# marcelodallaqua/TensorDiffEq

Measured on AMD Instinct MI355X. Metric: collocation-pts/sec + L2 rel-error, Allen-Cahn SA-PINN @ 1/2/4/8 GPU, higher is better.
Workload: dtype bf16; 1 GPU; model=Allen-Cahn SA-PINN tanh MLP [2,128,128,128,128,1], problem=ac-sa, global_batch=50000, parallelism=dp1, points_per_gpu=50000, backend=hip, bc_points=IC 512 (SA) + periodic 2x201 (u, u_x)

## Files before the change

tensordiffeq_amd/csrc/jet_bf3.hip:

```cpp
#include "jet_fused3.h"
#include "optim_common.h"

__device__ __forceinline__ void pack_frag(const float* __restrict__ P, bf16x8* __restrict__ img, const NetDims& d,
                                          int WT, int transposed, int e) {
  const int KB = WT / 2;
  {
    const int lane = e & 63, frag = e >> 6;
    const int kb = frag % KB, o = (frag / KB) % WT, layer = frag / (KB * WT) + 1;
    const int p = lane & 15, g = lane >> 4, row = 16 * o + p;
    const float* K = P + off_layer(d, layer);
    bf16x8 hi, lo;
#pragma unroll
    for (int j = 0; j < 8; ++j) {
      const int kf = 32 * kb + (j < 4 ? 4 * g + j : 16 + 4 * g + j - 4);
      const int in = transposed ? kf : row, out = transposed ? row : kf;
      const int win = hw(d, layer - 1), wout = hw(d, layer);
      const float v = (in < win && out < wout) ? K[in * wout + out] : 0.f;
      const __bf16 h = (__bf16)v;
      hi[j] = h;
      lo[j] = (__bf16)(v - (float)h);
    }
    img[(size_t)(frag * 2) * 64 + lane] = hi;
    img[(size_t)(frag * 2 + 1) * 64 + lane] = lo;
  }
}

__device__ __forceinline__ void pack_aux(const float* __restrict__ P, float* __restrict__ aux, const NetDims& d,
                                         int W, int e) {
  {
    float v = 0.f;
    const int w0 = hw(d, 0), wl = hw(d, d.n_hidden - 1);
    if (e < aux_b0(d, W)) {
      const int j = e / W, f = e - j * W;
      if (f < w0) v = P[j * w0 + f];
    } else if (e < aux_bh(d, W)) {
      const int f = e - aux_b0(d, W);
      if (f < w0) v = P[d.d_in * w0 + f];
    } else if (e < aux_ko(d, W)) {
      const int r = e - aux_bh(d, W), i = r / W + 1, f = r - (i - 1) * W;
      if (f < hw(d, i)) v = P[off_layer(d, i) + hw(d, i - 1) * hw(d, i) + f];
    } else if (e < aux_bo(d, W)) {
      const int r = e - aux_ko(d, W), f = r >> 2, q = r & 3;
      if (f < wl && q < d.d_out) v = P[off_layer(d, d.n_hidden) + f * d.d_out + q];
    } else {
      const int q = e - aux_bo(d, W);
      if (q < d.d_out) v = P[off_layer(d, d.n_hidden) + wl * d.d_out + q];
    }
    aux[e] = v;
  }
}

__global__ void __launch_bounds__(256) pack_all_kernel(const float* __restrict__ P, bf16x8* __restrict__ fimg,
                                                       bf16x8* __restrict__ bimg, float* __restrict__ aux, NetDims d,
                                                       int WT) {
  const int nf = (d.n_hidden - 1) * WT * (WT / 2) * 64;
  const int total = 2 * nf + aux_floats(d, 16 * WT);
  for (int e = blockIdx.x * 256 + threadIdx.x; e < total; e += gridDim.x * 256) {
    if (e < nf)
      pack_frag(P, fimg, d, WT, 1, e);
    else if (e < 2 * nf)
      pack_frag(P, bimg, d, WT, 0, e - nf);
    else
      pack_aux(P, aux, d, 16 * WT, e - 2 * nf);
  }
}

struct TailBook {
  const float* lpart;
  int n_lblocks, n_terms, n_scal;
  float* losses;
  float* total;
  float* dscal;
  float* hist;
  int64_t hist_rows;
  int64_t* epoch;
  float* best_loss;
  int64_t* best_epoch;
  int* improved;
  Counters cnt;
};

__global__ void __launch_bounds__(256) tail_reduce1_kernel(const float* __restrict__ slab, float* __restrict__ part,
                                                           int nwg, int Pst, int chunks, int nqb, int half, int c0,
                                                           TailBook tb) {
  if ((int)blockIdx.x < nqb) {
    const int q = blockIdx.x * 256 + threadIdx.x, c = c0 + (int)blockIdx.y;
    if (half) {
      if (8 * q < Pst) slab_reduce1_body8(slab, part, nwg, Pst, chunks, q, c);
    } else if (4 * q < Pst) {
      slab_reduce1_body<false>(slab, part, nwg, Pst, chunks, q, c);
    }
    return;
  }
  if (blockIdx.y != 0) return;
  __shared__ float sh[256];
  const int ns = tb.n_terms + tb.n_scal;
  for (int slot = 0; slot < ns; ++slot) {
    float s = 0.f;
    for (int b = threadIdx.x; b < tb.n_lblocks; b += 256) s += tb.lpart[(size_t)b * ns + slot];
    sh[threadIdx.x] = s;
    __syncthreads();
    for (int k = 128; k > 0; k >>= 1) {
      if ((int)threadIdx.x < k) sh[threadIdx.x] += sh[threadIdx.x + k];
      __syncthreads();
    }
    if (threadIdx.x == 0) {
      if (slot < tb.n_terms) tb.losses[slot] = sh[0];
      else tb.dscal[slot - tb.n_terms] = sh[0];
    }
    __syncthreads();
  }
  if (threadIdx.x == 0 && tb.hist == nullptr && tb.total != nullptr) {
    float s = 0.f;
    for (int t = 0; t < tb.n_terms; ++t) s += tb.losses[t];
    *tb.total = s;
  }
  if (threadIdx.x == 0 && tb.hist != nullptr)
    step_book_body(tb.total, tb.losses, tb.n_terms, 1, tb.hist, tb.hist_rows, tb.epoch, tb.best_loss, tb.best_epoch,
                   tb.improved, tb.cnt);
}

__global__ void __launch_bounds__(256) slab_reduce2_bf3(const float* __restrict__ part, float* __restrict__ grad, int P,
                                                        int Pst, int chunks, const float* __restrict__ gx) {
  const int q = blockIdx.x * 256 + threadIdx.x;
  if (4 * q >= P) return;
  const f32x4 a = slab_reduce2_sum(part, Pst, chunks, q);
#pragma unroll
  for (int e = 0; e < 4; ++e)
    if (4 * q + e < P) grad[4 * q + e] = gx != nullptr ? a[e] + gx[4 * q + e] : a[e];
}

__global__ void __launch_bounds__(256) tail_adam_kernel(AdamArgs args, const float* __restrict__ part, int Pst,
                                                        int chunks, const int* __restrict__ improved,
                                                        float* __restrict__ snap, TailImg ti,
                                                        const float* __restrict__ gx) {
  const bool do_snap = snap != nullptr && *improved != 0;
  const int64_t total = args.start[args.ngroups];
  for (int64_t idx = (int64_t)blockIdx.x * 256 + threadIdx.x; idx < total; idx += (int64_t)gridDim.x * 256) {
    const int gi = adam_group_of(args, idx);
    const AdamGroup gr = args.grp[gi];
    const int64_t e = idx - args.start[gi];
    const bool th = gi == 0;
    float g;
    if (th && part != nullptr) {
      float a0 = 0.f, a1 = 0.f;
      int c = 0;
      for (; c + 7 < chunks; c += 8) {
        float v[8];
#pragma unroll
        for (int k = 0; k < 8; ++k) v[k] = part[(size_t)(c + k) * Pst + e];
#pragma unroll
        for (int k = 0; k < 8; k += 2) {
          a0 += v[k];
          a1 += v[k + 1];
        }
      }
      for (; c + 1 < chunks; c += 2) {
        a0 += part[(size_t)c * Pst + e];
        a1 += part[(size_t)(c + 1) * Pst + e];
      }
      if (c < chunks) a0 += part[(size_t)c * Pst + e];
      g = a0 + a1;
      if (gx != nullptr) g += gx[e];
      const_cast<float*>(gr.g)[e] = g;
    } else {
      g = gr.g[e];
    }
    float p = gr.p[e], m = gr.m[e], v = gr.v[e];
    if (do_snap && th) snap[e] = p;
    adam_elem(p, gr.sign * g, m, v, gr.b1, gr.b2, gr.eps, adam_lr_t(gr));
    gr.p[e] = p;
    gr.m[e] = m;
    gr.v[e] = v;
    if (th && ti.fimg != nullptr) scatter_param(p, (int)e, ti);
  }
}

namespace {

int64_t img_floats(int WT, int n_hidden) {
  return (int64_t)(n_hidden > 1 ? n_hidden - 1 : 0) * WT * (WT / 2) * 128 * 4;
}

int64_t aux_alloc(int d_in, int n_hidden, int W) { return ((int64_t)(d_in + n_hidden + 4) * W + 4 + 3) / 4 * 4; }

int64_t stage_floats(int N, int WT, int S, int lo) {
  const int64_t nwg = (N + 63) / 64;
  return bf3_gstage(WT, S, lo != 0) ? nwg * 4 * stage_wave_elems(WT, S, true) * 2 : 0;
}

int bf3_rows(int N, const NetDims& d, int WT, int S, int lo) {
  const int pts_b = 16 * bwd_waves(WT, lo != 0, S);
  return (N + pts_b - 1) / pts_b;
}

int launch_pack(const float* P, bf16x8* fimg, bf16x8* bimg, float* aux, NetDims d, int WT, hipStream_t st) {
  const int total = 2 * (d.n_hidden - 1) * WT * (WT / 2) * 64 + aux_floats(d, 16 * WT);
  int blocks = (total + 255) / 256;
  if (blocks > 1024) blocks = 1024;
  hipLaunchKernelGGL(pack_all_kernel, dim3(blocks), dim3(256), 0, st, P, fimg, bimg, aux, d, WT);
  TDQ_CHECK_LAUNCH();
  return 0;
}

bool bf3_ok(int WT, int S, int d_in, int d_out, int n_hidden) {
  return (WT == 2 || WT == 4 || WT == 8 || (WT == 16 && S <= 4)) && S >= 1 && S <= TDQ_MAXS &&
         d_in <= TDQ_MAXD && d_out <= TDQ_MAXO && n_hidden >= 1;
}

int dispatch(bool fwd, int WT, int S, int nso, const Bf3Args& a) {
  switch (WT) {
    case 2: return fwd ? bf3_fwd_w2(S, nso, a) : bf3_bwd_w2(S, nso, a);
    case 4: return fwd ? bf3_fwd_w4(S, nso, a) : bf3_bwd_w4(S, nso, a);
    case 8: return fwd ? bf3_fwd_w8(S, nso, a) : bf3_bwd_w8(S, nso, a);
    case 16: return fwd ? bf3_fwd_w16(S, nso, a) : bf3_bwd_w16(S, nso, a);
    default: return (int)hipErrorInvalidValue;
  }
}

}

extern "C" {

int64_t tdq_jet_bf3_scratch_floats(int N, int d_in, const int* widths, int n_hidden, int S, int lo) {
  NetDims d;
  if (!make_dims(d, d_in, widths, 0, 1, n_hidden)) return -1;
  const int WT = width_tiles(d.width);
  if (WT < 2) return -1;
  const int64_t nwg = (N + 63) / 64;
  const int64_t hs = (int64_t)n_hidden * nwg * S * 4 * WT * 256;
  return hs + 2 * img_floats(WT, n_hidden) + aux_alloc(d_in, n_hidden, 16 * WT) + stage_floats(N, WT, S, lo);
}

int64_t tdq_jet_bf3_slab_floats(int N, int d_in, const int* widths, int d_out, int n_hidden) {
  NetDims d;
  if (!make_dims(d, d_in, widths, 0, d_out, n_hidden)) return -1;
  const int WT = width_tiles(d.width);
  if (WT < 2) return -1;
  int nwg = (N + 63) / 64;
  const int fz = (N + 15) / 16 < fz_cus() ? (N + 15) / 16 : fz_cus();
  if (fz > nwg) nwg = fz;
  const int64_t P = slab_stride(param_count(d));
  return ((int64_t)nwg + slab_chunks(nwg)) * P;
}

int64_t tdq_slab_floats_rows(int rows, int d_in, const int* widths, int d_out, int n_hidden) {
  NetDims d;
  if (rows < 1 || !make_dims(d, d_in, widths, 0, d_out, n_hidden)) return -1;
  return ((int64_t)rows + slab_chunks(rows)) * slab_stride(param_count(d));
}

static inline void scratch_images(float* scratch, int n_hidden, int WT, float** img, float** bimg, float** aux) {
  *img = scratch;
  *bimg = *img + img_floats(WT, n_hidden);
  *aux = *bimg + img_floats(WT, n_hidden);
}

static inline bf16x4* scratch_stage(float* scratch, int N, int d_in, int n_hidden, int S, int WT, int lo) {
  if (!bf3_gstage(WT, S, lo != 0)) return nullptr;
  float *img, *bimg, *aux;
  scratch_images(scratch, n_hidden, WT, &img, &bimg, &aux);
  return reinterpret_cast<bf16x4*>(aux + aux_alloc(d_in, n_hidden, 16 * WT));
}

static inline float* scratch_hs(float* scratch, int N, int d_in, int n_hidden, int S, int WT, int lo) {
  return scratch + 2 * img_floats(WT, n_hidden) + aux_alloc(d_in, n_hidden, 16 * WT) + stage_floats(N, WT, S, lo);
}

int tdq_jet_fwd_bf3_range(const float* X, const float* P, float* J, float* scratch, int N, int p_lo, int p_hi,
                          int d_in, const int* widths, int d_out, int n_hidden, int S, const int* spec, int lo, int pack,
                          void* stream) {
  if (N <= 0) return 0;
  if (p_lo < 0 || p_lo % 128 != 0 || p_hi > N || p_hi <= p_lo || (p_hi != N && p_hi % 128 != 0))
    return (int)hipErrorInvalidValue;
  NetDims d;
  if (!make_dims(d, d_in, widths, 0, d_out, n_hidden)) return (int)hipErrorInvalidValue;
  const int WT = width_tiles(d.width);
  JetSpec sp;
  if (!bf3_ok(WT, S, d_in, d_out, n_hidden)) return (int)hipErrorInvalidValue;
  const int nso = spec_nso(S, spec);
  if (nso < 0 || !make_spec(S, spec, sp)) return (int)hipErrorInvalidValue;
  hipStream_t st = reinterpret_cast<hipStream_t>(stream);
  float* Hs = scratch_hs(scratch, N, d_in, n_hidden, S, WT, lo);
  float *img, *bimg, *aux;
  scratch_images(scratch, n_hidden, WT, &img, &bimg, &aux);
  if (pack) {
    int rc = launch_pack(P, reinterpret_cast<bf16x8*>(img), reinterpret_cast<bf16x8*>(bimg), aux, d, WT, st);
    if (rc) return rc;
  }
  Bf3Args a{X, aux, reinterpret_cast<const bf16x8*>(img), nullptr, J, Hs, nullptr, N, 0, d, sp, st, lo,
            scratch_stage(scratch, N, d_in, n_hidden, S, WT, lo), p_lo, p_hi};
  return dispatch(true, WT, S, nso, a);
}

int tdq_jet_fwd_bf3_ex(const float* X, const float* P, float* J, float* scratch, int N, int d_in, const int* widths,
                       int d_out, int n_hidden, int S, const int* spec, int lo, int pack, void* stream) {
  return tdq_jet_fwd_bf3_range(X, P, J, scratch, N, 0, N, d_in, widths, d_out, n_hidden, S, spec, lo, pack, stream);
}

int tdq_jet_fwd_bf3(const float* X, const float* P, float* J, float* scratch, int N, int d_in, const int* widths,
                    int d_out, int n_hidden, int S, const int* spec, int lo, void* stream) {
  return tdq_jet_fwd_bf3_ex(X, P, J, scratch, N, d_in, widths, d_out, n_hidden, S, spec, lo, 1, stream);
}

int tdq_jet_bf3_pack(const float* P, float* scratch, int N, int d_in, const int* widths, int d_out, int n_hidden, int S,
                     void* stream) {
  NetDims d;
  if (!make_dims(d, d_in, widths, 0, d_out, n_hidden)) return (int)hipErrorInvalidValue;
  const int WT = width_tiles(d.width);
  if (!bf3_ok(WT, S, d_in, d_out, n_hidden)) return (int)hipErrorInvalidValue;
  float *img, *bimg, *aux;
  scratch_images(scratch, n_hidden, WT, &img, &bimg, &aux);
  return launch_pack(P, reinterpret_cast<bf16x8*>(img), reinterpret_cast<bf16x8*>(bimg), aux, d, WT,
                     reinterpret_cast<hipStream_t>(stream));
}

int tdq_jet_bwd_bf3_range(const float* X, const float* dJ, const float* Hs, float* work, int N, int p_lo, int p_hi,
                          int d_in, const int* widths, int d_out, int n_hidden, int S, const int* spec, int lo,
                          void* stream) {
  if (N <= 0) return 0;
  if (p_lo < 0 || p_lo % 128 != 0 || p_hi > N || p_hi <= p_lo || (p_hi != N && p_hi % 128 != 0))
    return (int)hipErrorInvalidValue;
  NetDims d;
  if (!make_dims(d, d_in, widths, 0, d_out, n_hidden)) return (int)hipErrorInvalidValue;
  const int WT = width_tiles(d.width);
  JetSpec sp;
  if (!bf3_ok(WT, S, d_in, d_out, n_hidden)) return (int)hipErrorInvalidValue;
  const int nso = spec_nso(S, spec);
  if (nso < 0 || !make_spec(S, spec, sp)) return (int)hipErrorInvalidValue;
  hipStream_t st = reinterpret_cast<hipStream_t>(stream);
  const int Ptot = param_count(d);
  float* scr = const_cast<float*>(Hs);
  float *img, *bimg, *aux;
  scratch_images(scr, n_hidden, WT, &img, &bimg, &aux);
  Bf3Args a{X, aux, reinterpret_cast<const bf16x8*>(bimg), dJ, nullptr, scratch_hs(scr, N, d_in, n_hidden, S, WT, lo),
            work, N, slab_stride(Ptot), d, sp, st, lo, scratch_stage(scr, N, d_in, n_hidden, S, WT, lo), p_lo, p_hi};
  return dispatch(false, WT, S, nso, a);
}

int tdq_jet_bwd_bf3_ex(const float* X, const float* P, const float* dJ, const float* Hs, float* work, float* grad,
                       int N, int d_in, const int* widths, int d_out, int n_hidden, int S, const int* spec, int lo, int reduce,
                       void* stream) {
  if (N <= 0) return 0;
  (void)P;
  int rc = tdq_jet_bwd_bf3_range(X, dJ, Hs, work, N, 0, N, d_in, widths, d_out, n_hidden, S, spec, lo, stream);
  if (rc || !reduce) return rc;
  NetDims d;
  make_dims(d, d_in, widths, 0, d_out, n_hidden);
  const int WT = width_tiles(d.width);
  const int nwg_b = bf3_rows(N, d, WT, S, lo);
  const int Ptot = param_count(d);
  return tdq_slab_reduce_h(work, grad, nwg_b, Ptot, slab_chunks(nwg_b), (int)slab_half(lo != 0), stream);
}

int tdq_jet_bwd_bf3(const float* X, const float* P, const float* dJ, const float* Hs, float* work, float* grad,
                    int N, int d_in, const int* widths, int d_out, int n_hidden, int S, const int* spec, int lo,
                    void* stream) {
  return tdq_jet_bwd_bf3_ex(X, P, dJ, Hs, work, grad, N, d_in, widths, d_out, n_hidden, S, spec, lo, 1, stream);
}

int tdq_step_tail_bf3(float* work, float* grad, float* scratch, int N, int d_in, const int* widths, int d_out, int n_hidden,
                      int S, int lo, const float* lpart, int n_lblocks, int n_terms, int n_scal, float* losses,
                      float* total, float* dscal, float* hist, int64_t hist_rows, int64_t* epoch, float* best_loss,
                      int64_t* best_epoch, int* improved, double* const* counters, int ncnt, const void* groups,
                      int ngroups, float* snap, int c_first, const float* gx, int rows, void* stream) {
  NetDims d;
  if (!make_dims(d, d_in, widths, 0, d_out, n_hidden)) return (int)hipErrorInvalidValue;
  const int WT = width_tiles(d.width);
  if (!bf3_ok(WT, S, d_in, d_out, n_hidden) || ncnt < 0 || ncnt > TDQ_MAX_COUNTERS || n_lblocks < 0 ||
      n_terms < 0 || n_scal < 0)
    return (int)hipErrorInvalidValue;
  AdamArgs args;
  if (!adam_args_fill(args, reinterpret_cast<const AdamGroup*>(groups), ngroups, true))
    return (int)hipErrorInvalidValue;
  const int Ptot = param_count(d);
  if (args.grp[0].n != Ptot) return (int)hipErrorInvalidValue;
  args.grp[0].g = grad;
  hipStream_t st = reinterpret_cast<hipStream_t>(stream);
  const int nwg_b = rows > 0 ? rows : bf3_rows(N, d, WT, S, lo);
  const int Pst = slab_stride(Ptot), chunks = slab_chunks(nwg_b);
  if (c_first < 0 || c_first >= chunks) return (int)hipErrorInvalidValue;
  float* part = work + (size_t)nwg_b * Pst;
  TailBook tb;
  tb.lpart = lpart;
  tb.n_lblocks = n_lblocks;
  tb.n_terms = n_terms;
  tb.n_scal = n_scal;
  tb.losses = losses;
  tb.total = total;
  tb.dscal = dscal;
  tb.hist = hist;
  tb.hist_rows = hist_rows;
  tb.epoch = epoch;
  tb.best_loss = best_loss;
  tb.best_epoch = best_epoch;
  tb.improved = improved;
  tb.cnt.n = ncnt;
  for (int i = 0; i < TDQ_MAX_COUNTERS; ++i) tb.cnt.c[i] = i < ncnt ? counters[i] : nullptr;
  const int half = (int)slab_half(lo != 0);
  const int nqb = (Pst / (half ? 8 : 4) + 255) / 256;
  hipLaunchKernelGGL(tail_reduce1_kernel, dim3(nqb + 1, chunks - c_first), dim3(256), 0, st, work, part, nwg_b, Pst,
                     chunks, nqb, half, c_first, tb);
  TDQ_CHECK_LAUNCH();
  TailImg ti{nullptr, nullptr, nullptr, d, WT};
  if (scratch != nullptr) {
    float *img, *bimg, *aux;
    scratch_images(scratch, n_hidden, WT, &img, &bimg, &aux);
    ti.fimg = reinterpret_cast<__bf16*>(img);
    ti.bimg = reinterpret_cast<__bf16*>(bimg);
    ti.aux = aux;
  }
  const int64_t tot = args.start[ngroups];
  int64_t blocks = (tot + 255) / 256;
  if (blocks > 2048) blocks = 2048;
  if (blocks < 1) blocks = 1;
  hipLaunchKernelGGL(tail_adam_kernel, dim3((unsigned)blocks), dim3(256), 0, st, args, part, Pst, chunks, improved,
                     snap, ti, gx);
  TDQ_CHECK_LAUNCH();
  return 0;
}

int tdq_dp_tail_a_bf3(float* work, float* grad, int N, int d_in, const int* widths, int d_out, int n_hidden, int S, int lo,
                      const float* lpart, int n_lblocks, int n_terms, int n_scal, float* losses, float* dscal,
                      float* total, int c_first, const float* gx, int rows, int half_ovr, void* stream) {
  NetDims d;
  if (!make_dims(d, d_in, widths, 0, d_out, n_hidden)) return (int)hipErrorInvalidValue;
  const int WT = width_tiles(d.width);
  if (!bf3_ok(WT, S, d_in, d_out, n_hidden) || N < 1 || n_lblocks < 0 || n_terms < 0 || n_scal < 0)
    return (int)hipErrorInvalidValue;
  hipStream_t st = reinterpret_cast<hipStream_t>(stream);
  const int Ptot = param_count(d);
  const int nwg_b = rows > 0 ? rows : bf3_rows(N, d, WT, S, lo);
  const int Pst = slab_stride(Ptot), chunks = slab_chunks(nwg_b);
  if (c_first < 0 || c_first >= chunks) return (int)hipErrorInvalidValue;
  float* part = work + (size_t)nwg_b * Pst;
  TailBook tb{};
  tb.lpart = lpart;
  tb.n_lblocks = n_lblocks;
  tb.n_terms = n_terms;
  tb.n_scal = n_scal;
  tb.losses = losses;
  tb.dscal = dscal;
  tb.total = total;
  const int half = half_ovr >= 0 ? (half_ovr != 0) : (int)slab_half(lo != 0);
  const int nqb = (Pst / (half ? 8 : 4) + 255) / 256, nq2 = (Pst / 4 + 255) / 256;
  hipLaunchKernelGGL(tail_reduce1_kernel, dim3(nqb + 1, chunks - c_first), dim3(256), 0, st, work, part, nwg_b, Pst,
                     chunks, nqb, half, c_first, tb);
  TDQ_CHECK_LAUNCH();
  hipLaunchKernelGGL(slab_reduce2_bf3, dim3(nq2), dim3(256), 0, st, part, grad, Ptot, Pst, chunks, gx);
  TDQ_CHECK_LAUNCH();
  return 0;
}

int tdq_bf3_slab_geometry(int N, int d_in, const int* widths, int d_out, int n_hidden, int S, int lo, int* out) {
  NetDims d;
  if (!make_dims(d, d_in, widths, 0, d_out, n_hidden)) return (int)hipErrorInvalidValue;
  const int WT = width_tiles(d.width);
  if (!bf3_ok(WT, S, d_in, d_out, n_hidden) || N < 1) return (int)hipErrorInvalidValue;
  const int pts_b = 16 * bwd_waves(WT, lo != 0, S), nwg_b = bf3_rows(N, d, WT, S, lo),
            chunks = slab_chunks(nwg_b);
  out[0] = pts_b;
  out[1] = nwg_b;
  out[2] = chunks;
  out[3] = 0;
  return 0;
}

int tdq_slab_prereduce_bf3(float* work, int N, int d_in, const int* widths, int d_out, int n_hidden, int S, int lo,
                           int c0, int c1, void* stream) {
  NetDims d;
  if (!make_dims(d, d_in, widths, 0, d_out, n_hidden)) return (int)hipErrorInvalidValue;
  const int WT = width_tiles(d.width);
  if (!bf3_ok(WT, S, d_in, d_out, n_hidden) || N < 1) return (int)hipErrorInvalidValue;
  const int Ptot = param_count(d);
  const int nwg_b = bf3_rows(N, d, WT, S, lo);
  const int Pst = slab_stride(Ptot), chunks = slab_chunks(nwg_b);
  if (c0 < 0 || c1 > chunks || c1 <= c0) return (int)hipErrorInvalidValue;
  float* part = work + (size_t)nwg_b * Pst;
  const int half = (int)slab_half(lo != 0);
  const int nqb = (Pst / (half ? 8 : 4) + 255) / 256;
  TailBook tb{};
  hipLaunchKernelGGL(tail_reduce1_kernel, dim3(nqb, c1 - c0), dim3(256), 0, reinterpret_cast<hipStream_t>(stream),
                     work, part, nwg_b, Pst, chunks, nqb, half, c0, tb);
  TDQ_CHECK_LAUNCH();
  return 0;
}

int tdq_dp_tail_b_bf3(float* scratch, int N, int d_in, const int* widths, int d_out, int n_hidden, int S,
                      const void* groups, int ngroups, const int* improved, float* snap, void* stream) {
  NetDims d;
  if (!make_dims(d, d_in, widths, 0, d_out, n_hidden)) return (int)hipErrorInvalidValue;
  const int WT = width_tiles(d.width);
  if (!bf3_ok(WT, S, d_in, d_out, n_hidden)) return (int)hipErrorInvalidValue;
  AdamArgs args;
  if (!adam_args_fill(args, reinterpret_cast<const AdamGroup*>(groups), ngroups, true))
    return (int)hipErrorInvalidValue;
  if (args.grp[0].n != param_count(d)) return (int)hipErrorInvalidValue;
  TailImg ti{nullptr, nullptr, nullptr, d, WT};
  if (scratch != nullptr) {
    float *img, *bimg, *aux;
    scratch_images(scratch, n_hidden, WT, &img, &bimg, &aux);
    ti.fimg = reinterpret_cast<__bf16*>(img);
    ti.bimg = reinterpret_cast<__bf16*>(bimg);
    ti.aux = aux;
  }
  const int64_t tot = args.start[ngroups];
  int64_t blocks = (tot + 255) / 256;
  if (blocks > 2048) blocks = 2048;
  if (blocks < 1) blocks = 1;
  hipLaunchKernelGGL(tail_adam_kernel, dim3((unsigned)blocks), dim3(256), 0, reinterpret_cast<hipStream_t>(stream),
                     args, nullptr, 0, 0, improved, snap, ti, nullptr);
  TDQ_CHECK_LAUNCH();
  return 0;
}

int tdq_fused_step_launch(void* func, const float* X, float* scratch, float* work, int N, int d_in, const int* widths,
                          int d_out, int n_hidden, int S, const int* spec, int G, const void* lptrs,
                          float* lpart, int prow, int nacc, int lo, void* stream) {
  if (func == nullptr || N <= 0 || G < 1 || prow < 0 || nacc < 1 || lo < 0 || lo > 1)
    return (int)hipErrorInvalidValue;
  NetDims d;
  if (!make_dims(d, d_in, widths, 0, d_out, n_hidden)) return (int)hipErrorInvalidValue;
  const int WT = width_tiles(d.width);
  if (!bf3_ok(WT, S, d_in, d_out, n_hidden) || tdq_jet_fused_lds(d_in, widths, d_out, n_hidden, S, lo) < 0)
    return (int)hipErrorInvalidValue;
  const int PT = lo ? FZ3_PT : FZ_PT;
  if (G > (N + PT - 1) / PT) return (int)hipErrorInvalidValue;
  JetSpec sp;
  if (spec_nso(S, spec) < 0 || !make_spec(S, spec, sp)) return (int)hipErrorInvalidValue;
  float *img, *bimg, *aux;
  scratch_images(scratch, n_hidden, WT, &img, &bimg, &aux);
  FzParams P{};
  P.X = X;
  P.aux = aux;
  P.fimg = reinterpret_cast<const bf16x8*>(img);
  P.bimg = reinterpret_cast<const bf16x8*>(bimg);
  P.slab = work;
  P.N = N;
  P.Pst = slab_stride(param_count(d));
  P.ntiles = (N + PT - 1) / PT;
  P.d = d;
  P.lptrs = reinterpret_cast<const FzLossPtrs*>(lptrs);
  P.lpart = lpart;
  P.prow = prow;
  P.nacc = nacc;
  void* args[] = {(void*)&P};
  return (int)hipModuleLaunchKernel((hipFunction_t)func, (unsigned)G, 1, 1, 64 * FZ_WAVES, 1, 1, 0,
                                    reinterpret_cast<hipStream_t>(stream), args, nullptr);
}

int tdq_fused_params_size() { return (int)sizeof(FzParams); }

int tdq_img_target(float* scratch, int d_in, const int* widths, int d_out, int n_hidden, void* out, int out_bytes) {
  NetDims d;
  if (scratch == nullptr || out == nullptr || !make_dims(d, d_in, widths, 0, d_out, n_hidden)) return -1;
  const int WT = width_tiles(d.width);
  if (WT < 2 || out_bytes < (int)sizeof(TailImg)) return -1;
  float *img, *bimg, *aux;
  scratch_images(scratch, n_hidden, WT, &img, &bimg, &aux);
  TailImg ti{reinterpret_cast<__bf16*>(img), reinterpret_cast<__bf16*>(bimg), aux, d, WT};
  *reinterpret_cast<TailImg*>(out) = ti;
  return (int)sizeof(TailImg);
}

}
```

tensordiffeq_amd/csrc/jet_fused.h:

```cpp
#pragma once
#include "jet_bf3.h"

#ifndef FZ_TS_TILE
#define FZ_TS_TILE 0
#endif
#define FZ_TS(k) \
  do {                \
    if (t == t0 + FZ_TS_TILE) TDQ_TS(k); \
  } while (0)

#define FZ_PT 32
#define FZ_WAVES 8

__host__ __device__ constexpr int fz_nslot(int LM) { return LM < 2 ? 2 : LM; }
__host__ __device__ constexpr int fz_img_elems(int WT, int S, int LM) {
  return (S + 1) * fz_nslot(LM) * FZ_PT * bf3_img_rs(WT);
}
struct FzFl {
  int bh, ko, bo, xs, ubs, part, pq, outp, lpre, total;
};
__host__ __device__ constexpr FzFl fz_fl(int W, int d_in, int S, int LM, int PT, int NQ, int NW) {
  FzFl f{};
  f.bh = (d_in + 1) * W;
  f.ko = (d_in + LM + 1) * W;
  f.bo = (d_in + LM + 5) * W;
  f.xs = (f.bo + 4 + 3) / 4 * 4;
  f.ubs = f.xs + PT * TDQ_MAXD;
  f.part = f.ubs + S * PT * 4;
  f.pq = (LM + 1) * W + d_in * W + 4 * W;
  f.outp = f.part + NQ * f.pq + 4;
  f.lpre = f.outp + NW * S * PT;
  f.total = f.lpre + PT;
  return f;
}
__host__ __device__ inline int fz_lds_bytes(const NetDims& d, int WT, int S, int LM) {
  return fz_img_elems(WT, S, LM) * 2 + fz_fl(16 * WT, d.d_in, S, LM, FZ_PT, 2, 4).total * 4;
}

template <int WT, int S, int NSO, bool CHEAP, int DIN>
__device__ __forceinline__ void fz_h0(const JetSpec& sp, const float* aux, const float* xrow, int t, int g,
                                      f32x4 (&h)[S]) {
  constexpr int S1 = S - 1 - NSO, SO = 1 + S1, W = 16 * WT;
  static_assert(DIN > 0, "fz_h0: compile-time input width");
  const int f0 = 16 * t + 4 * g;
  f32x4 z = *reinterpret_cast<const f32x4*>(aux + DIN * W + f0);
  {
    float x[DIN];
#pragma unroll
    for (int j = 0; j < DIN; ++j) x[j] = xrow[j];
#pragma unroll
    for (int c = 0; c < 4; ++c) {
      float a = z[c];
#pragma unroll
      for (int j = 0; j < DIN; ++j) a = fmaf(x[j], aux[j * W + f0 + c], a);
      z[c] = a;
    }
  }
  f32x4 ka[S];
  ka[0] = zero4();
#pragma unroll
  for (int s = 1; s < SO; ++s) ka[s] = *reinterpret_cast<const f32x4*>(aux + sp.var[s] * W + f0);
#pragma unroll
  for (int s = SO; s < S; ++s) ka[s] = zero4();
  f32x4 kp[S];
#pragma unroll
  for (int s = SO; s < S; ++s) kp[s] = sel_first<S, S1>(ka, sp.ia[s], sp.selA[s]) * sel_first<S, S1>(ka, sp.ib[s], sp.selB[s]);
#pragma unroll
  for (int c = 0; c < 4; ++c) {
    float hv, s1;
    if constexpr (CHEAP) {
      const float e = __builtin_amdgcn_exp2f(fminf(z[c], 15.f) * 2.8853900817779268f);
      const float r = __builtin_amdgcn_rcpf(1.f + e);
      hv = fmaf(-2.f, r, 1.f);
      s1 = (4.f * e) * (r * r);
    } else {
      tanh_s1(z[c], hv, s1);
    }
    const float s2 = -2.f * hv * s1;
    h[0][c] = hv;
#pragma unroll
    for (int s = 1; s < SO; ++s) h[s][c] = s1 * ka[s][c];
#pragma unroll
    for (int s = SO; s < S; ++s) h[s][c] = s2 * kp[s][c];
  }
}

struct FzLane {
  int lo, r2;
};
template <int RS>
__device__ __forceinline__ FzLane fz_lane(int p, int g) {
  const int ch = g ^ ((p >> 2) & 3), rsw = (p & 8) << 3;
  return FzLane{p * RS + 4 * ch + rsw, 2 * rsw};
}
template <int RS>
__device__ __forceinline__ int fz_at(const FzLane& L, int q, int t) {
  return L.lo - ((t >> 2) & 1) * L.r2 + 16 * q * RS + 16 * t;
}
template <int RS>
__device__ __forceinline__ void fz_put(__bf16* im, const FzLane& L, int q, int t, bf16x4 v) {
  *reinterpret_cast<bf16x4*>(im + fz_at<RS>(L, q, t)) = v;
}
template <int RS>
__device__ __forceinline__ bf16x4 fz_get(const __bf16* im, const FzLane& L, int q, int t) {
  return *reinterpret_cast<const bf16x4*>(im + fz_at<RS>(L, q, t));
}
template <int RS>
__device__ __forceinline__ bf16x8 fz_bfrag(const __bf16* im, const FzLane& L, int q, int kb) {
  return cat8(fz_get<RS>(im, L, q, 2 * kb), fz_get<RS>(im, L, q, 2 * kb + 1));
}
__device__ __forceinline__ f32x4 fz_bf4(bf16x4 v) {
  const u32x2 u = __builtin_bit_cast(u32x2, v);
  return f32x4{__uint_as_float(u[0] << 16), __uint_as_float(u[0] & 0xffff0000u), __uint_as_float(u[1] << 16),
               __uint_as_float(u[1] & 0xffff0000u)};
}
template <int WT, int S>
__device__ __forceinline__ void fz_get_h(const __bf16* im, const FzLane& L, int q, int t, f32x4 (&h)[S]) {
  constexpr int RS = bf3_img_rs(WT), SIMG = FZ_PT * RS;
  h[0] = fz_bf4(fz_get<RS>(im, L, q, t)) + fz_bf4(fz_get<RS>(im + S * SIMG, L, q, t));
#pragma unroll
  for (int s = 1; s < S; ++s) h[s] = fz_bf4(fz_get<RS>(im + s * SIMG, L, q, t));
}

template <int WT, int OPW>
struct FzW {
  bf16x8 a[WT / 2][OPW];
};
constexpr int FZ_WAHEAD = 2;
template <int WT, int OPW>
__device__ __forceinline__ void fz_load_w(FzW<WT, OPW>& w, const bf16x8* __restrict__ wimg, int layer, int o0, int l,
                                          int kb) {
  constexpr int KB = WT / 2, NSTEP = WT * KB;
  if (kb >= KB) return;
  const Tl Wi = tl_make(wimg + (size_t)(layer - 1) * NSTEP * 128, l);
#pragma unroll
  for (int oo = 0; oo < OPW; ++oo) {
    bf16x8 unused;
    img_frag<false>(Wi, (o0 + oo) * KB + kb, w.a[kb][oo], unused);
  }
}
template <int WT, int OPW>
__device__ __forceinline__ void fz_pre_w(FzW<WT, OPW>& w, const bf16x8* __restrict__ wimg, int layer, int o0, int l) {
#pragma unroll
  for (int kb = 0; kb < FZ_WAHEAD; ++kb) fz_load_w<WT, OPW>(w, wimg, layer, o0, l, kb);
}

template <int WT, int S, int OPW>
__device__ __forceinline__ void fz_gemm(f32x4 (&acc)[OPW][S], FzW<WT, OPW>& w, const bf16x8* __restrict__ wimg, int layer,
                                        int o0, int l, const __bf16* im, int q, const FzLane& L) {
  constexpr int KB = WT / 2, RS = bf3_img_rs(WT), SIMG = FZ_PT * RS;
#pragma unroll
  for (int oo = 0; oo < OPW; ++oo)
#pragma unroll
    for (int s = 0; s < S; ++s) acc[oo][s] = zero4();
#pragma unroll
  for (int kb = 0; kb < KB; ++kb) {
    fz_load_w<WT, OPW>(w, wimg, layer, o0, l, kb + FZ_WAHEAD);
    bf16x8 b[S];
#pragma unroll
    for (int s = 0; s < S; ++s) b[s] = fz_bfrag<RS>(im + s * SIMG, L, q, kb);
#pragma unroll
    for (int oo = 0; oo < OPW; ++oo)
#pragma unroll
      for (int s = 0; s < S; ++s) acc[oo][s] = mfma_bf(w.a[kb][oo], b[s], acc[oo][s]);
    __builtin_amdgcn_sched_barrier(0);
  }
}

struct FzTr {
  int a1, a2, z1, z2;
};
template <int RS, int NR, int NC>
__device__ __forceinline__ FzTr fz_tr(int r0, int c0, int l) {
  const int g = l >> 4;
  const int tr_row = 8 * g + ((l & 15) >> 2);
  const int swz = (g & 1) << 6;
  const int tr_col1 = 4 * ((l & 3) ^ ((2 * g) & 3)), tr_col2 = 4 * ((l & 3) ^ ((2 * g + 1) & 3));
  static_assert((NR == 4 || NR <= 2) && (NC == 4 || NC <= 2), "fz_tr: tile blocks of 1, 2 or 4");
  return FzTr{tr_row * RS + tr_col1 + ((16 * r0) ^ swz), (tr_row + 4) * RS + tr_col2 + ((16 * r0) ^ swz),
              tr_row * RS + tr_col1 + ((16 * c0) ^ swz), (tr_row + 4) * RS + tr_col2 + ((16 * c0) ^ swz)};
}
template <int WT, int S, int NR, int NC, bool SB = true, int SIMG = FZ_PT * bf3_img_rs(WT)>
__device__ __forceinline__ void fz_dk(f32x4 (&dk)[NR][NC], const __bf16* H, const __bf16* Z, int r0, int c0, int l) {
  const auto [a1, a2, z1, z2] = fz_tr<bf3_img_rs(WT), NR, NC>(r0, c0, l);
#pragma unroll
  for (int s = 0; s < S; ++s) {
    bf16x8 A[NR], B[NC];
#pragma unroll
    for (int r = 0; r < NR; ++r) A[r] = cat8(tr_read(H + s * SIMG + a1 + 16 * r), tr_read(H + s * SIMG + a2 + 16 * r));
#pragma unroll
    for (int c = 0; c < NC; ++c) B[c] = cat8(tr_read(Z + s * SIMG + z1 + 16 * c), tr_read(Z + s * SIMG + z2 + 16 * c));
#pragma unroll
    for (int r = 0; r < NR; ++r)
#pragma unroll
      for (int c = 0; c < NC; ++c) dk[r][c] = mfma_bf(A[r], B[c], dk[r][c]);
    if constexpr (SB) __builtin_amdgcn_sched_barrier(0);
  }
}

struct FzLossPtrs {
  const float* val[16];
  const float* lam[8];
  float* dlam[8];
  const float* scal[8];
};

struct FzParams {
  const float* X;
  const float* aux;
  const bf16x8* fimg;
  const bf16x8* bimg;
  float* slab;
  int N, Pst, ntiles;
  NetDims d;
  const FzLossPtrs* lptrs;
  float* lpart;
  int prow, nacc;
};

template <int S, int PT, int NW>
__device__ __forceinline__ float fz_jsum(const float* jv, int s, int k, float bo) {
  float a = jv[s * PT + k];
#pragma unroll
  for (int w = 1; w < NW; ++w) a += jv[(w * S + s) * PT + k];
  return s == 0 ? a + bo : a;
}


template <int PT>
__device__ __forceinline__ void fz_stage(float* xs, float* lpre, int tid, float v) {
  if (tid < PT * TDQ_MAXD) xs[tid] = v;
  else if (tid < PT * TDQ_MAXD + PT) lpre[tid - PT * TDQ_MAXD] = v;
}

template <int WT, int LM, int NAUX>
__device__ __forceinline__ void fz_setup(const FzParams& P, float* aux, int tid) {
  const float* __restrict__ aux_g = P.aux;
  const int G = gridDim.x, gi = blockIdx.x;
  bf16x8 wpf[2];
  {
    constexpr int NI16 = LM * WT * (WT / 2) * 128 * 4 * 4 / 16;
    const int xw = gi >> 3, nx = (G + 7) >> 3;
#pragma unroll
    for (int k = 0; k < 2; ++k) {
      const int e = (xw + k * nx) * 64 * FZ_WAVES + tid;
      wpf[k] = e < 2 * NI16 ? (e < NI16 ? P.fimg[e] : P.bimg[e - NI16]) : bf16x8{};
    }
  }
  for (int e = tid; e < NAUX; e += 64 * FZ_WAVES) aux[e] = e < aux_floats(P.d, 16 * WT) ? aux_g[e] : 0.f;
  asm volatile("" ::"v"(wpf[0]), "v"(wpf[1]));
}

template <int WT, int S, int NSO, int LM, class LossF>
__device__ __forceinline__ void fz_body(const FzParams& P, char* lds_raw) {
  const int N = P.N, Pst = P.Pst, ntiles = P.ntiles;
  const NetDims& d = P.d;
  constexpr JetSpec sp = LossF::SPEC;
  constexpr int DIN = LossF::DIN;
  constexpr int W = 16 * WT, OPW = WT / 4, RS = bf3_img_rs(WT), SIMG = FZ_PT * RS, PT = FZ_PT;
  constexpr int NR = WT / 4, NC = WT / 2;
  constexpr int ZS = 0;
  static_assert(OPW >= 1 && OPW * 4 == WT, "fused step: WT = 4 or 8");
  static_assert(LM >= 2, "fused step keeps h_LM in h_0's slot");
  __bf16* img = reinterpret_cast<__bf16*>(lds_raw);
  auto slot = [&](int k) { return img + k * (S + 1) * SIMG; };
  constexpr FzFl F = fz_fl(W, DIN, S, LM, PT, 2, 4);
  float* aux = reinterpret_cast<float*>(img + fz_img_elems(WT, S, LM));
  float *xs = aux + F.xs, *ubs = aux + F.ubs, *part = aux + F.part, *outp = aux + F.outp, *lpre = aux + F.lpre;

  const int tid = threadIdx.x, l = tid & 63, p = l & 15, g = l >> 4;
  const int w = __builtin_amdgcn_readfirstlane(tid >> 6);
  const int q = w >> 2, wo = w & 3;
  const int G = gridDim.x, gi = blockIdx.x;
  const int t0 = (int)((long long)ntiles * gi / G), t1 = (int)((long long)ntiles * (gi + 1) / G);
  const int r0 = NR * (w >> 1), c0 = NC * (w & 1);
  const int o0 = wo * OPW;
  const int row = 16 * q + p;
  const FzLane L = fz_lane<RS>(p, g);
  float* accB = part + q * F.pq;
  float* accK0 = accB + (LM + 1) * W;
  float* accKo = accK0 + DIN * W;
  const bf16x8* Wimg = P.fimg;
  const bf16x8* Kimg = P.bimg;

  static_assert(FZ_PT * TDQ_MAXD + FZ_PT <= 64 * FZ_WAVES, "one element per thread");
  const float* __restrict__ X = P.X;
  float xpre = 0.f;
  auto fetch = [&](int tt) {
    const int pb = tt * FZ_PT;
    if (tid < FZ_PT * TDQ_MAXD) {
      const int pt = tid / TDQ_MAXD, j = tid - pt * TDQ_MAXD;
      const int n = min(pb + pt, N - 1);
      xpre = j < DIN ? X[(size_t)n * DIN + j] : 0.f;
    } else if (tid < FZ_PT * TDQ_MAXD + FZ_PT) {
      xpre = LossF::pre(pb + tid - FZ_PT * TDQ_MAXD, N, *P.lptrs);
    }
  };
  if (t0 < t1) fetch(t0);
  fz_setup<WT, LM, F.xs>(P, aux, tid);
  f32x4 dk[LM][NR][NC];
  float lacc[LossF::NACC];
  float bo_acc = 0.f;
#pragma unroll
  for (int k = 0; k < LossF::NACC; ++k) lacc[k] = 0.f;
#pragma unroll
  for (int i = 0; i < LM; ++i)
#pragma unroll
    for (int r = 0; r < NR; ++r)
#pragma unroll
      for (int c = 0; c < NC; ++c) dk[i][r][c] = zero4();
  for (int e = tid; e < 2 * F.pq + 4; e += 64 * FZ_WAVES) part[e] = 0.f;
  const float* Ko = aux + F.ko;

  auto layer0 = [&](int oo, f32x4(&h)[S]) { fz_h0<WT, S, NSO, true, DIN>(sp, aux, xs + row * TDQ_MAXD, o0 + oo, g, h); };

  int t = t0;
  FzW<WT, OPW> wf;
  TDQ_TS(0);
  while (t < t1) {
    const int pb = t * PT;
    asm volatile("" : "+s"(Wimg), "+s"(Kimg));
    __syncthreads();
    fz_stage<PT>(xs, lpre, tid, xpre);
    if (t + 1 < t1) fetch(t + 1);
    __syncthreads();
    FZ_TS(1);

#pragma unroll
    for (int oo = 0; oo < OPW; ++oo) {
      f32x4 h[S];
      layer0(oo, h);
#pragma unroll
      for (int s = 0; s < S; ++s) fz_put<RS>(slot(0) + s * SIMG, L, q, o0 + oo, cvt_hi4(h[s]));
    }
    fz_pre_w<WT, OPW>(wf, Wimg, 1, o0, l);
    __syncthreads();
    FZ_TS(2);

#pragma unroll
    for (int ly = 1; ly <= LM; ++ly) {
      const float* bi = aux + F.bh + (ly - 1) * W;
      f32x4 acc[OPW][S];
      fz_gemm<WT, S, OPW>(acc, wf, Wimg, ly, o0, l, slot(ly - 1), q, L);
      FZ_TS(1 + 2 * ly);
      f32x4 hq[OPW][S];
#pragma unroll
      for (int oo = 0; oo < OPW; ++oo) {
        const int to = o0 + oo;
        f32x4 z[S], h[S];
#pragma unroll
        for (int s = 0; s < S; ++s) z[s] = acc[oo][s];
        z[0] += *reinterpret_cast<const f32x4*>(bi + 16 * to + 4 * g);
        tanh_jet_f<S, NSO>(sp, z, h);
        __bf16* im = slot(ly < LM ? ly : ZS);
        bf16x4 hi, lo;
        split4(h[0], hi, lo);
        fz_put<RS>(im, L, q, to, hi);
        fz_put<RS>(im + S * SIMG, L, q, to, lo);
#pragma unroll
        for (int s = 1; s < S; ++s) fz_put<RS>(im + s * SIMG, L, q, to, cvt_hi4(h[s]));
        if (ly == LM) {
#pragma unroll
          for (int s = 0; s < S; ++s) hq[oo][s] = h[s];
        }
      }
      if (ly == LM) {
#pragma unroll
        for (int s = 0; s < S; ++s) {
          float a = 0.f;
#pragma unroll
          for (int oo = 0; oo < OPW; ++oo)
#pragma unroll
            for (int c = 0; c < 4; ++c) a = fmaf(hq[oo][s][c], Ko[(16 * (o0 + oo) + 4 * g + c) * 4], a);
          const float r = col4_sum(a);
          if (g == 0) outp[(wo * S + s) * FZ_PT + row] = r;
        }
      }
      if (ly < LM) fz_pre_w<WT, OPW>(wf, Wimg, ly + 1, o0, l);
      __syncthreads();
      FZ_TS(2 + 2 * ly);
    }

    int tl = tid;
    asm volatile("" : "+v"(tl));
    if (tl < PT) LossF::template eval<S, PT, 4>(outp, xs, tl, pb + tl, N, *P.lptrs, ubs, lacc, lpre[tl], aux[F.bo]);
    __syncthreads();
    FZ_TS(9);
    tl = tid;
    asm volatile("" : "+v"(tl));
    if (tl < PT) bo_acc += ubs[tl * 4];
#pragma unroll
    for (int oo = 0; oo < OPW; ++oo) {
      const int to = o0 + oo;
      __bf16* im = slot(ZS);
      f32x4 h[S], hb[S], zb[S];
      fz_get_h<WT, S>(im, L, q, to, h);
      f32x4 kq, pp = zero4();
#pragma unroll
      for (int c = 0; c < 4; ++c) kq[c] = Ko[(16 * to + 4 * g + c) * 4];
#pragma unroll
      for (int s = 0; s < S; ++s) {
        const float ub = ubs[(s * FZ_PT + row) * 4];
        hb[s] = kq * ub;
        pp += h[s] * ub;
      }
      {
        const float r = row16_sum4(pp);
        if ((p & 3) == 0) accKo[(16 * to + 4 * g + (p >> 2)) * 4] += r;
      }
      tanh_jet_b<S, NSO>(sp, h, hb, zb);
      const float r = row16_sum4(zb[0]);
      if ((p & 3) == 0) accB[LM * W + 16 * to + 4 * g + (p >> 2)] += r;
#pragma unroll
      for (int s = 0; s < S; ++s) fz_put<RS>(im + s * SIMG, L, q, to, cvt_hi4(zb[s]));
    }
    fz_pre_w<WT, OPW>(wf, Kimg, LM, o0, l);
    __syncthreads();
#pragma unroll
    for (int ly = LM; ly >= 1; --ly) {
      const __bf16* Z = slot(ly == LM ? ZS : ly);
      __bf16* H = slot(ly - 1);
      const int tb = 10 + 5 * (LM - ly);
      f32x4 acc[OPW][S];
      fz_gemm<WT, S, OPW>(acc, wf, Kimg, ly, o0, l, Z, q, L);
      FZ_TS(tb);
      bf16x4 zbh[OPW][S];
      float rb[OPW];
      if (ly >= 2) {
#pragma unroll
        for (int oo = 0; oo < OPW; ++oo) {
          const int to = o0 + oo;
          f32x4 h[S], zb[S];
          fz_get_h<WT, S>(H, L, q, to, h);
          tanh_jet_b<S, NSO>(sp, h, acc[oo], zb);
          rb[oo] = row16_sum4(zb[0]);
#pragma unroll
          for (int s = 0; s < S; ++s) zbh[oo][s] = cvt_hi4(zb[s]);
        }
      }
      fz_dk<WT, S, NR, NC, false>(dk[ly - 1], H, Z, r0, c0, l);
      FZ_TS(tb + 1);
      if (ly >= 2) {
        __syncthreads();
        FZ_TS(tb + 2);
#pragma unroll
        for (int oo = 0; oo < OPW; ++oo) {
          const int to = o0 + oo;
          if ((p & 3) == 0) accB[(ly - 1) * W + 16 * to + 4 * g + (p >> 2)] += rb[oo];
#pragma unroll
          for (int s = 0; s < S; ++s) fz_put<RS>(H + s * SIMG, L, q, to, zbh[oo][s]);
        }
      } else {
#pragma unroll
        for (int oo = 0; oo < OPW; ++oo) {
          const int to = o0 + oo;
          f32x4 h[S], zb[S];
          fz_get_h<WT, S>(H, L, q, to, h);
          tanh_jet_b<S, NSO>(sp, h, acc[oo], zb);
          const int fo = 16 * to + 4 * g + (p >> 2);
          {
            const float r = row16_sum4(zb[0]);
            if ((p & 3) == 0) accB[fo] += r;
          }
#pragma unroll
          for (int j = 0; j < DIN; ++j) {
            const float xj = xs[row * TDQ_MAXD + j];
            f32x4 vv;
#pragma unroll
            for (int c = 0; c < 4; ++c) {
              float a = xj * zb[0][c];
              constexpr int SO = S - NSO;
#pragma unroll
              for (int s = 1; s < SO; ++s) a += (sp.var[s] == j) ? zb[s][c] : 0.f;
              vv[c] = a;
            }
            const float r = row16_sum4(vv);
            if ((p & 3) == 0) accK0[j * W + fo] += r;
          }
        }
      }
      FZ_TS(tb + 3);
      if (ly == 2) {
        if (LM == 2) __syncthreads();
#pragma unroll
        for (int oo = 0; oo < OPW; ++oo) {
          f32x4 h[S];
          layer0(oo, h);
          bf16x4 hi, lo;
          split4(h[0], hi, lo);
          fz_put<RS>(slot(0), L, q, o0 + oo, hi);
          fz_put<RS>(slot(0) + S * SIMG, L, q, o0 + oo, lo);
#pragma unroll
          for (int s = 1; s < S; ++s) fz_put<RS>(slot(0) + s * SIMG, L, q, o0 + oo, cvt_hi4(h[s]));
        }
      }
      if (ly >= 2) {
        fz_pre_w<WT, OPW>(wf, Kimg, ly - 1, o0, l);
        __syncthreads();
      }
      FZ_TS(tb + 4);
    }
    ++t;
  }
  TDQ_TS(62);

  __bf16* gs = reinterpret_cast<__bf16*>(P.slab) + (size_t)gi * Pst;
#pragma unroll
  for (int ly = 1; ly <= LM; ++ly) {
    const int voff = ((16 * r0 + 4 * g) * W + 16 * c0 + p) * 2;
    const Tl Gt = tl_make(gs + off_layer(d, ly), 0);
#pragma unroll
    for (int r = 0; r < NR; ++r)
#pragma unroll
      for (int c = 0; c < NC; ++c)
#pragma unroll
        for (int e = 0; e < 4; ++e)
          __builtin_amdgcn_raw_buffer_store_b16(__builtin_bit_cast(unsigned short, (__bf16)dk[ly - 1][r][c][e]),
                                                Gt.r, voff, ((16 * r + e) * W + 16 * c) * 2, 0);
  }
  __syncthreads();
  const float* pA = part;
  const float* pB = part + F.pq;
  for (int f = tid; f < W; f += 64 * FZ_WAVES) {
    gs[DIN * W + f] = (__bf16)(pA[f] + pB[f]);
    for (int ly = 1; ly <= LM; ++ly)
      gs[off_layer(d, ly) + W * W + f] = (__bf16)(pA[ly * W + f] + pB[ly * W + f]);
    for (int j = 0; j < DIN; ++j) {
      const int k = (LM + 1) * W + j * W + f;
      gs[j * W + f] = (__bf16)(pA[k] + pB[k]);
    }
    for (int qo = 0; qo < d.d_out; ++qo) {
      const int k = (LM + 1 + DIN) * W + f * 4 + qo;
      gs[off_layer(d, LM + 1) + f * d.d_out + qo] = (__bf16)(pA[k] + pB[k]);
    }
  }
  if (w == 0) {
    const float bo = col4_sum(row16_sum(bo_acc));
    if (l == 0) gs[off_layer(d, LM + 1) + W] = (__bf16)bo;
#pragma unroll
    for (int k = 0; k < LossF::NACC; ++k) {
      const float v = col4_sum(row16_sum(lacc[k]));
      if (l == 0 && k < P.nacc) P.lpart[(size_t)(P.prow + gi) * P.nacc + k] = v;
    }
  }
  TDQ_TS(63);
}

#ifndef __HIPCC_RTC__
int fz_cus();
extern "C" int tdq_jet_fused_lds(int d_in, const int* widths, int d_out, int n_hidden, int S, int lo);
#endif
```

Before: 372.5 million collocation-pts/s.

## Stage per-block gradient slab in LDS and write it with coalesced 16-byte stores

Each block's bf16 gradient slab, weights plus bias and output partials, is first assembled in the freed LDS image area using a padded row layout. Lane pairs are combined with DPP and perm so each thread writes 32-bit values. The slab is then copied to global memory with 16-byte vector stores instead of scattered 2-byte buffer stores. The goal is to cut the kernel epilogue's global-write transaction count. In exchange it adds extra barriers, a possible chunked path when LDS is too small, and host-side layout and alignment checks that reject unsupported configurations.

```diff
diff --git a/tensordiffeq_amd/csrc/jet_bf3.hip b/tensordiffeq_amd/csrc/jet_bf3.hip
--- a/tensordiffeq_amd/csrc/jet_bf3.hip
+++ b/tensordiffeq_amd/csrc/jet_bf3.hip
@@ -538,6 +538,11 @@
   P.slab = work;
   P.N = N;
   P.Pst = slab_stride(param_count(d));
+  for (int ly = 1; ly <= n_hidden; ++ly)
+    if (off_layer(d, ly) != fz_off(d_in, d.width, ly)) return (int)hipErrorInvalidValue;
+  if (param_count(d) != fz_params(d_in, d.width, n_hidden - 1) || P.Pst % 8 != 0 ||
+      reinterpret_cast<uintptr_t>(work) % 16 != 0)
+    return (int)hipErrorInvalidValue;
   P.ntiles = (N + PT - 1) / PT;
   P.d = d;
   P.lptrs = reinterpret_cast<const FzLossPtrs*>(lptrs);
diff --git a/tensordiffeq_amd/csrc/jet_fused.h b/tensordiffeq_amd/csrc/jet_fused.h
--- a/tensordiffeq_amd/csrc/jet_fused.h
+++ b/tensordiffeq_amd/csrc/jet_fused.h
@@ -8,6 +8,10 @@
   do {                \
     if (t == t0 + FZ_TS_TILE) TDQ_TS(k); \
   } while (0)
+
+#ifndef FZ_SLAB_FORM
+#define FZ_SLAB_FORM -1
+#endif
 
 #define FZ_PT 32
 #define FZ_WAVES 8
@@ -251,6 +255,55 @@
   asm volatile("" ::"v"(wpf[0]), "v"(wpf[1]));
 }
 
+__host__ __device__ constexpr int fz_off(int DIN, int W, int ly) { return (DIN + 1) * W + (ly - 1) * (W * W + W); }
+__host__ __device__ constexpr int fz_params(int DIN, int W, int LM) { return fz_off(DIN, W, LM + 1) + W + 1; }
+template <class T, int W>
+__host__ __device__ constexpr int fz_row_at(int x) {
+  return x + (16 / (int)sizeof(T)) * (x / W);
+}
+template <class T>
+__host__ __device__ constexpr int fz_row_form(int bytes, int DIN, int W, int LM) {
+  const int pad = 16 / (int)sizeof(T), layer = W * W + W;
+  const int whole = fz_params(DIN, W, LM), first = (DIN + 1) * W + layer, last = layer + W + 1;
+  const int chunk = first > last ? first : last;
+  const int cap = bytes / (int)sizeof(T);
+  return whole + pad * (whole / W + 1) <= cap ? 2 : chunk + pad * (chunk / W + 1) <= cap ? 1 : 0;
+}
+template <int RS, int NR, int NC>
+__device__ __forceinline__ void fz_row_put_dk(__bf16* st, const f32x4 (&dk)[NR][NC], int r0, int c0, int p, int g) {
+  const bool odd = p & 1;
+  __bf16* b = st + (16 * r0 + 4 * g + (odd ? 2 : 0)) * RS + 16 * c0 + (p & ~1);
+  const unsigned keep = odd ? 0x03020706u : 0x05040100u;
+#pragma unroll
+  for (int r = 0; r < NR; ++r)
+#pragma unroll
+    for (int c = 0; c < NC; ++c)
+#pragma unroll
+      for (int e = 0; e < 2; ++e) {
+        const unsigned own = __builtin_bit_cast(unsigned, bf16x2{(__bf16)dk[r][c][e], (__bf16)dk[r][c][e + 2]});
+        const unsigned nb = (unsigned)__builtin_amdgcn_update_dpp(0, (int)own, 0xB1, 0xF, 0xF, false);
+        *reinterpret_cast<unsigned*>(b + (16 * r + e) * RS + 16 * c) = __builtin_amdgcn_perm(nb, own, keep);
+      }
+}
+template <class T, int W, int MAXN>
+__device__ __forceinline__ void fz_row_copy(const T* st, T* gs, int lo, int hi, int tid) {
+  constexpr int E = 16 / (int)sizeof(T), NT = 64 * FZ_WAVES, NIT = (MAXN / E + NT - 1) / NT;
+  const int ng = (hi - lo) / E;
+  u32x4 v[NIT];
+#pragma unroll
+  for (int i = 0; i < NIT; ++i) {
+    const int j = tid + i * NT;
+    if (j < ng) v[i] = *reinterpret_cast<const u32x4*>(st + fz_row_at<T, W>(E * j));
+  }
+#pragma unroll
+  for (int i = 0; i < NIT; ++i) {
+    const int j = tid + i * NT;
+    if (j < ng) *reinterpret_cast<u32x4*>(gs + lo + E * j) = v[i];
+  }
+  const int x = ng * E + tid;
+  if (x < hi - lo) gs[lo + x] = st[fz_row_at<T, W>(x)];
+}
+
 template <int WT, int S, int NSO, int LM, class LossF>
 __device__ __forceinline__ void fz_body(const FzParams& P, char* lds_raw) {
   const int N = P.N, Pst = P.Pst, ntiles = P.ntiles;
@@ -504,43 +557,84 @@
   }
   TDQ_TS(62);
 
+  int tq = tid;
+  asm volatile("" : "+v"(tq));
+  const int ge = (tq >> 4) & 3;
   __bf16* gs = reinterpret_cast<__bf16*>(P.slab) + (size_t)gi * Pst;
-#pragma unroll
-  for (int ly = 1; ly <= LM; ++ly) {
-    const int voff = ((16 * r0 + 4 * g) * W + 16 * c0 + p) * 2;
-    const Tl Gt = tl_make(gs + off_layer(d, ly), 0);
-#pragma unroll
-    for (int r = 0; r < NR; ++r)
-#pragma unroll
-      for (int c = 0; c < NC; ++c)
-#pragma unroll
-        for (int e = 0; e < 4; ++e)
-          __builtin_amdgcn_raw_buffer_store_b16(__builtin_bit_cast(unsigned short, (__bf16)dk[ly - 1][r][c][e]),
-                                                Gt.r, voff, ((16 * r + e) * W + 16 * c) * 2, 0);
-  }
-  __syncthreads();
+  constexpr int FORM = FZ_SLAB_FORM < 0 ? fz_row_form<__bf16>(fz_img_elems(WT, S, LM) * 2, DIN, W, LM) : FZ_SLAB_FORM;
+  static_assert(FORM <= fz_row_form<__bf16>(fz_img_elems(WT, S, LM) * 2, DIN, W, LM), "the staged form fits the image area");
   const float* pA = part;
   const float* pB = part + F.pq;
-  for (int f = tid; f < W; f += 64 * FZ_WAVES) {
-    gs[DIN * W + f] = (__bf16)(pA[f] + pB[f]);
-    for (int ly = 1; ly <= LM; ++ly)
-      gs[off_layer(d, ly) + W * W + f] = (__bf16)(pA[ly * W + f] + pB[ly * W + f]);
-    for (int j = 0; j < DIN; ++j) {
-      const int k = (LM + 1) * W + j * W + f;
-      gs[j * W + f] = (__bf16)(pA[k] + pB[k]);
-    }
-    for (int qo = 0; qo < d.d_out; ++qo) {
-      const int k = (LM + 1 + DIN) * W + f * 4 + qo;
-      gs[off_layer(d, LM + 1) + f * d.d_out + qo] = (__bf16)(pA[k] + pB[k]);
-    }
+  const float bo = w == 0 ? col4_sum(row16_sum(bo_acc)) : 0.f;
+  if constexpr (FORM != 0) {
+    constexpr int NCH = FORM == 2 ? 1 : LM, NP = fz_params(DIN, W, LM);
+    constexpr int MAXN = FORM == 2 ? NP : (DIN + 2) * W + W * W + W + 1;
+    __syncthreads();
+#pragma unroll
+    for (int ch = 0; ch < NCH; ++ch) {
+      const int l0 = FORM == 2 ? 1 : ch + 1, l1 = FORM == 2 ? LM : ch + 1;
+      const int lo = ch == 0 ? 0 : fz_off(DIN, W, l0), hi = ch == NCH - 1 ? NP : fz_off(DIN, W, l1 + 1);
+      auto at = [&](int x) { return img + fz_row_at<__bf16, W>(x - lo); };
+      if (ch > 0) __syncthreads();
+#pragma unroll
+      for (int ly = 1; ly <= LM; ++ly)
+        if (ly >= l0 && ly <= l1)
+          fz_row_put_dk<fz_row_at<__bf16, W>(W), NR, NC>(at(fz_off(DIN, W, ly)), dk[ly - 1], r0, c0, p, ge);
+      for (int f = tid; f < W; f += 64 * FZ_WAVES) {
+        if (ch == 0) {
+          *at(DIN * W + f) = (__bf16)(pA[f] + pB[f]);
+          for (int j = 0; j < DIN; ++j) {
+            const int k = (LM + 1) * W + j * W + f;
+            *at(j * W + f) = (__bf16)(pA[k] + pB[k]);
+          }
+        }
+        for (int ly = l0; ly <= l1; ++ly)
+          *at(fz_off(DIN, W, ly) + W * W + f) = (__bf16)(pA[ly * W + f] + pB[ly * W + f]);
+        if (ch == NCH - 1) {
+          const int k = (LM + 1 + DIN) * W + f * 4;
+          *at(fz_off(DIN, W, LM + 1) + f) = (__bf16)(pA[k] + pB[k]);
+        }
+      }
+      if (ch == NCH - 1 && tid == 0) *at(fz_off(DIN, W, LM + 1) + W) = (__bf16)bo;
+      __syncthreads();
+      if (ch == NCH - 1) TDQ_TS(61);
+      fz_row_copy<__bf16, W, MAXN>(img, gs, lo, hi, tid);
+    }
+  } else {
+#pragma unroll
+    for (int ly = 1; ly <= LM; ++ly) {
+      const int voff = ((16 * r0 + 4 * ge) * W + 16 * c0 + p) * 2;
+      const Tl Gt = tl_make(gs + off_layer(d, ly), 0);
+#pragma unroll
+      for (int r = 0; r < NR; ++r)
+#pragma unroll
+        for (int c = 0; c < NC; ++c)
+#pragma unroll
+          for (int e = 0; e < 4; ++e)
+            __builtin_amdgcn_raw_buffer_store_b16(__builtin_bit_cast(unsigned short, (__bf16)dk[ly - 1][r][c][e]),
+                                                  Gt.r, voff, ((16 * r + e) * W + 16 * c) * 2, 0);
+    }
+    __syncthreads();
+    for (int f = tid; f < W; f += 64 * FZ_WAVES) {
+      gs[DIN * W + f] = (__bf16)(pA[f] + pB[f]);
+      for (int ly = 1; ly <= LM; ++ly)
+        gs[off_layer(d, ly) + W * W + f] = (__bf16)(pA[ly * W + f] + pB[ly * W + f]);
+      for (int j = 0; j < DIN; ++j) {
+        const int k = (LM + 1) * W + j * W + f;
+        gs[j * W + f] = (__bf16)(pA[k] + pB[k]);
+      }
+      for (int qo = 0; qo < d.d_out; ++qo) {
+        const int k = (LM + 1 + DIN) * W + f * 4 + qo;
+        gs[off_layer(d, LM + 1) + f * d.d_out + qo] = (__bf16)(pA[k] + pB[k]);
+      }
+    }
+    if (tid == 0) gs[off_layer(d, LM + 1) + W] = (__bf16)bo;
   }
   if (w == 0) {
-    const float bo = col4_sum(row16_sum(bo_acc));
-    if (l == 0) gs[off_layer(d, LM + 1) + W] = (__bf16)bo;
 #pragma unroll
     for (int k = 0; k < LossF::NACC; ++k) {
       const float v = col4_sum(row16_sum(lacc[k]));
-      if (l == 0 && k < P.nacc) P.lpart[(size_t)(P.prow + gi) * P.nacc + k] = v;
+      if ((tid & 63) == 0 && k < P.nacc) P.lpart[(size_t)(P.prow + gi) * P.nacc + k] = v;
     }
   }
   TDQ_TS(63);
```

New measurement: 375.5 million collocation-pts/s (median of 6 runs). No clear change (+0.8%).
